# prstrive/SCGaussian

Hardware: AMD Instinct MI355X
Metric: train_iters_per_sec (higher is better)
Workload: dtype f32; 1 GPU; S2: 200000 Gaussians, 1008x756, SH degree 3, fwd+bwd per view (BASELINE configs[1] shape: LLFF-fern 3-view training, 200 k Gaussians @ 1008x756); gaussians=200000, width=1008, height=756, sh_degree=3, visible=174771, views=3, parallelism=single, ranks_seen=1, launched_by=single process, grad_bucket_bytes=0, grad_bucket_bytes_per_view=0

## Files before the change

### include/scg_raster.h

```cpp
#ifndef SCG_RASTER_H
#define SCG_RASTER_H

#include <stddef.h>
#include <stdint.h>

#ifndef SCG_API
#define SCG_API __attribute__((visibility("default")))
#endif

#ifdef __cplusplus
extern "C" {
#endif

#define SCG_TILE 16
#define SCG_SPLAT_FLOATS 12
#define SCG_DSPLAT_FLOATS 16
#define SCG_ABI_VERSION 10

enum {
    SCG_OK = 0,
    SCG_E_NULL = -1,
    SCG_E_RANGE = -2,
    SCG_E_EXCLUSIVE = -3,
    SCG_E_SCRATCH = -4,
// ... 1 lines not shown
};

typedef struct ScgFrame {
    int32_t P;
    int32_t sh_degree;
    int32_t sh_coeffs;
    int32_t width;
    int32_t height;
    float tanfovx;
    float tanfovy;
    float scale_modifier;
    int32_t prefiltered;
    int32_t debug;
    const float* viewmatrix;
    const float* projmatrix;
    const float* campos;
    const float* bg;
    const uint32_t* tile_cost_in;
    uint32_t* tile_cost_out;
    uint32_t* long_lists_out;
    const uint32_t* bwd_cost_in;
    uint32_t* bwd_cost_out;
    uint32_t* num_rendered_out;
} ScgFrame;


SCG_API const char* scg_last_error(void);
SCG_API int32_t scg_abi_version(void);
SCG_API size_t scg_struct_bytes(int32_t which );

SCG_API size_t scg_geometry_scratch_bytes(int32_t P);
SCG_API int scg_geometry_forward(const ScgFrame* frame,
                         const float* means3D, const float* opacities,
                         const float* shs, const float* colors_precomp,
                         const float* scales, const float* rotations, const float* cov3D_precomp,
                         float* splats, int32_t* radii, uint8_t* clamped,
                         uint32_t* rects, uint32_t* depth_keys, uint32_t* num_rendered_out,
                         void* scratch, size_t scratch_bytes, void* stream);

enum { SCG_BINNING_AUTO = 0, SCG_BINNING_GLOBAL_SORT = 1 };
SCG_API size_t scg_binning_scratch_bytes(int32_t P, int64_t num_rendered, int32_t width, int32_t height, int32_t algo);
SCG_API size_t scg_ranges_words(int32_t width, int32_t height);
SCG_API int32_t scg_binning_accepts_bound(int64_t num_rendered_bound, int32_t width, int32_t height, int32_t algo);
SCG_API int scg_binning(const ScgFrame* frame, int64_t num_rendered,
                const uint32_t* rects, const uint32_t* depth_keys,
                uint32_t* point_list, uint32_t* ranges, uint64_t* keys_sorted, int32_t algo,
// ... 160 lines not shown
```

### scgaussian_amd/_lib.py

```python
from __future__ import annotations

import ctypes as C
import os

import torch

_HERE = os.path.dirname(os.path.abspath(__file__))
LIB_PATH = os.environ.get("SCG_LIB_PATH") or os.path.join(_HERE, "libscg_raster.so")

ABI_VERSION = 10


class ScgFrame(C.Structure):
    _fields_ = [
        ("P", C.c_int32), ("sh_degree", C.c_int32), ("sh_coeffs", C.c_int32),
        ("width", C.c_int32), ("height", C.c_int32),
        ("tanfovx", C.c_float), ("tanfovy", C.c_float), ("scale_modifier", C.c_float),
        ("prefiltered", C.c_int32), ("debug", C.c_int32),
        ("viewmatrix", C.c_void_p), ("projmatrix", C.c_void_p), ("campos", C.c_void_p), ("bg", C.c_void_p),
        ("tile_cost_in", C.c_void_p), ("tile_cost_out", C.c_void_p), ("long_lists_out", C.c_void_p),
        ("bwd_cost_in", C.c_void_p), ("bwd_cost_out", C.c_void_p), ("num_rendered_out", C.c_void_p),
    ]


class ScgWorkspaceLayout(C.Structure):
    _fields_ = [(n, C.c_uint64) for n in ("splats", "rects", "depth_keys", "clamped", "point_list", "ranges", "final_T",
                                          "n_contrib", "bin_scratch", "total", "partial_words")]


class ScgStageEvents(C.Structure):
    _fields_ = [("begin", C.c_void_p * 3), ("end", C.c_void_p * 3)]


class ScgModelSet(C.Structure):
    _fields_ = [("count", C.c_int32)] + [(n, C.c_void_p) for n in ("zval", "rayo", "rayd", "xyz", "features_dc", "features_rest",
                                                                   "opacity", "scaling", "rotation")]


class ScgModel(C.Structure):
    _fields_ = [("ray", ScgModelSet), ("bg", ScgModelSet)]


class ScgModelGradSet(C.Structure):
    _fields_ = [(n, C.c_void_p) for n in ("zval", "xyz", "features_dc", "features_rest", "opacity", "scaling", "rotation")]
# ... 107 lines not shown
```

### scgaussian_amd/csrc/api.hip

```cpp
#include <stdarg.h>
#include <stdio.h>
#include <string.h>

#include "scg_common.h"
#include "scg_debug.h"

#include <atomic>
#include <chrono>
#include <thread>

namespace scg {

static thread_local char g_err[512] = "";

int fail(int code, const char* fmt, ...) {
    va_list ap;
    va_start(ap, fmt);
    vsnprintf(g_err, sizeof(g_err), fmt, ap);
    va_end(ap);
    return code;
}

int check_hip(hipError_t e, const char* what) {
    if (e == hipSuccess) return 0;
    snprintf(g_err, sizeof(g_err), "%s: %s (hipError %d)", what, hipGetErrorString(e), (int)e);
    return (int)e;
}

int validate_frame(const ScgFrame* f, bool need_bg) {
    if (!f) return fail(SCG_E_NULL, "frame is NULL");
    if (f->P < 0) return fail(SCG_E_RANGE, "P = %d < 0", f->P);
    if (f->width <= 0 || f->height <= 0 || f->width > 65535 * SCG_TILE || f->height > 65535 * SCG_TILE)
        return fail(SCG_E_RANGE, "image size %d x %d out of range", f->width, f->height);
    if (f->sh_degree < 0 || f->sh_degree > 3) return fail(SCG_E_RANGE, "sh_degree %d not in 0..3", f->sh_degree);
    if (!(f->tanfovx > 0.f) || !(f->tanfovy > 0.f)) return fail(SCG_E_RANGE, "tanfov must be positive");
    if (!f->viewmatrix || !f->projmatrix || !f->campos) return fail(SCG_E_NULL, "viewmatrix/projmatrix/campos is NULL");
    if (need_bg && !f->bg) return fail(SCG_E_NULL, "bg is NULL");
    return 0;
}

static inline size_t align_up(size_t v, size_t a) { return (v + a - 1) / a * a; }
static inline bool aligned16(const void* p) { return (reinterpret_cast<uintptr_t>(p) & 15u) == 0; }
static inline bool aligned64(const void* p) { return (reinterpret_cast<uintptr_t>(p) & 63u) == 0; }
int validate_model(const ScgFrame* f, const ScgModel* m);

static int validate_inputs(const ScgFrame* f, const float* means3D, const float* opacities, const float* shs,
                           const float* colors_precomp, const float* scales, const float* rotations,
                           const float* cov3D_precomp) {
    if (f->P == 0) return 0;
    if (!means3D || !opacities) return fail(SCG_E_NULL, "means3D/opacities is NULL");
    if ((shs == nullptr) == (colors_precomp == nullptr))
        return fail(SCG_E_EXCLUSIVE, "Please provide exactly one of either SHs or precomputed colors!");
    const bool has_sr = scales != nullptr && rotations != nullptr;
    if ((scales != nullptr) != (rotations != nullptr) || has_sr == (cov3D_precomp != nullptr))
        return fail(SCG_E_EXCLUSIVE,
                    "Please provide exactly one of either scale/rotation pair or precomputed 3D covariance!");
    if (shs && f->sh_coeffs < (f->sh_degree + 1) * (f->sh_degree + 1))
        return fail(SCG_E_RANGE, "sh_coeffs %d < (sh_degree+1)^2 = %d", f->sh_coeffs,
                    (f->sh_degree + 1) * (f->sh_degree + 1));
    if (rotations && !aligned16(rotations)) return fail(SCG_E_ALIGN, "rotations must be 16-byte aligned");
// ... 534 lines not shown
```

### scgaussian_amd/csrc/blend.hip

```cpp
#include "scg_common.h"
#include "tile_sort.h"

namespace scg {

constexpr float kHalfLog2e = 0.72134752044448170f;
typedef float f32x2 __attribute__((ext_vector_type(2)));
typedef float f32x4 __attribute__((ext_vector_type(4)));

__device__ __forceinline__ bool splat_hits_rect(const float4& a, const float4& b, float x0, float y0) {
    const float dx0 = x0 - a.x, dy0 = y0 - a.y, dx1 = dx0 + 7.0f, dy1 = dy0 + 7.0f;
    const float nx = __builtin_amdgcn_fmed3f(0.0f, dx0, dx1), ny = __builtin_amdgcn_fmed3f(0.0f, dy0, dy1);
    const float cb2 = a.w + a.w;
    const float ya = __builtin_amdgcn_fmed3f(b.w * nx, dy0, dy1);
    const float qa = nx * (a.z * nx + cb2 * ya) + b.x * ya * ya;
    const float xb = __builtin_amdgcn_fmed3f(-a.w * ny * __builtin_amdgcn_rcpf(a.z), dx0, dx1);
    const float qb = ny * (b.x * ny + cb2 * xb) + a.z * xb * xb;
    return !((qa > b.z) && (qb > b.z));
}

__device__ __forceinline__ int quadrant_workgroup(int wg, int n_tiles, const uint2* __restrict__ ranges, int& quad) {
    quad = (wg >> 3) & 3;
    const int per = (n_tiles + 7) >> 3;
    const uint32_t* order = reinterpret_cast<const uint32_t*>(ranges) + 2 * (size_t)n_tiles;
    return (int)order[(wg & 7) * per + (wg >> 5)];
// ... 11 lines not shown
                                             const float4* __restrict__ splats, float* __restrict__ out_color,
                                             float* __restrict__ out_depth, float* __restrict__ out_alpha,
                                             float* __restrict__ final_T, uint32_t* __restrict__ n_contrib) {
    const int tile_x = tile % f.gx, tile_y = tile / f.gx;
    const int qx0 = tile_x * kTile + (quad & 1) * 8, qy0 = tile_y * kTile + (quad >> 1) * 8;
    const int px = qx0 + (lane & 7), py = qy0 + (lane >> 3);
    const bool inside = (px < f.W) && (py < f.H);
    const float pxf = (float)px, pyf = (float)py;

    const int n = (int)(range.y - range.x);
    float T = inside ? 1.0f : -1.0f;
    int bgi0 = __builtin_amdgcn_readfirstlane(__builtin_bit_cast(int, f.bg[0]));
    int bgi1 = __builtin_amdgcn_readfirstlane(__builtin_bit_cast(int, f.bg[1]));
    int bgi2 = __builtin_amdgcn_readfirstlane(__builtin_bit_cast(int, f.bg[2]));
    asm volatile("" : "+s"(bgi0), "+s"(bgi1), "+s"(bgi2));
    f32x2 Crg = {0.f, 0.f}, Cbz = {0.f, 0.f};
    uint32_t last = 0;
    int n_blended = 0;
#ifndef SCG_FWD_TRIP_CXX
    const uint32_t lds_base = (uint32_t)reinterpret_cast<uintptr_t>(s_rec);
    const uint64_t exec_all = __builtin_amdgcn_read_exec();
#endif

    uint32_t id_next = 0;
    float4 ra, rb, rc;
    if (n > 0) {
        const uint32_t id0 = list[min(lane, n - 1)];
        id_next = list[min(kWave + lane, n - 1)];
        ra = splats[3 * (size_t)id0 + 0]; rb = splats[3 * (size_t)id0 + 1]; rc = splats[3 * (size_t)id0 + 2];
    }

    for (int base = 0; base < n; base += kWave) {
        if (__all(T < 0.0f)) break;
        const bool hit = (base + lane < n) && splat_hits_rect(ra, rb, (float)qx0, (float)qy0);
        if (hit) {
            *reinterpret_cast<float2*>(&s_rec[2 * kWave + lane]) = make_float2(ra.x, ra.y);
            s_rec[kWave + lane] = make_float4(kHalfLog2e * ra.z, 2.0f * kHalfLog2e * ra.w, kHalfLog2e * rb.x, rb.y);
            s_rec[lane] = rc;
        }
        uint64_t m = __ballot(hit);
        if (base + kWave < n) {
            ra = splats[3 * (size_t)id_next + 0]; rb = splats[3 * (size_t)id_next + 1];
            rc = splats[3 * (size_t)id_next + 2];
            id_next = list[min(base + 2 * kWave + lane, n - 1)];
        }
        wave_sync();

        n_blended += __builtin_popcountll(m);
#ifdef SCG_FWD_TRIP_CXX
        while (m) {
            const int j = __builtin_ctzll(m);
            asm("s_bitset0_b64 %0, %1" : "+s"(m) : "s"(j));
            const float2 c = *reinterpret_cast<const float2*>(&s_rec[2 * kWave + j]);
            const float4 q = s_rec[kWave + j];
            const float dx = c.x - pxf, dy = c.y - pyf;
            const float u = __builtin_fmaf(q.y, dy, q.x * dx);
            const float t = __builtin_fmaf(u, dx, (q.z * dy) * dy);
            const float alpha = fminf(kAlphaMax, q.w * __builtin_amdgcn_exp2f(-t));
            const float wgt = T * alpha;
            const float test_T = __builtin_fmaf(-T, alpha, T);
            if ((t >= 0.0f) && (alpha >= kAlphaMin)) {
                const bool contributes = test_T >= kTEps;
                const float T_prev = T;
// ... 245 lines not shown
        "v_cndmask_b32 %1, %3, %4, %20\n\t"
        "s_nop 1\n\t"
        "v_add_f32_dpp %0, %1, %5 quad_perm:[2,3,0,1] row_mask:0xf bank_mask:0xf"
        : "=&v"(y), "=&v"(t0), "=&v"(t1), "=&v"(t2), "=&v"(t3), "=&v"(t4), "=&v"(t5), "=&v"(t6), "=&v"(t7)
        : "v"(v0), "v"(v1), "v"(v2), "v"(v3), "v"(v4), "v"(v5), "v"(v6), "v"(v7), "v"(v8), "v"(v9), "s"(odd), "s"(hi));
    return y;
}

struct BwdLds {
    float4 a[kWave];
    float4 b[kWave];
    float4 c[kWave];
    __attribute__((aligned(16))) float w[kSlots * kWStride];
};

struct BwdPixel {
    float T, behind, dC0, dC1, dC2, dD, dA;
    uint32_t last;
};

__device__ __forceinline__ uint32_t top_chunk_index(int end) {
    return (uint32_t)min(((end - 1) / kWave) * kWave + (kWave - 1 - (int)threadIdx.x), end - 1);
}
__device__ __forceinline__ int backward_walk(BwdLds& L, const FrameDev& f, int tile, int quad, int first, int end,
                                              BwdPixel px, uint32_t list_begin, uint32_t id_top,
                                              const uint32_t* __restrict__ point_list,
                                              const float4* __restrict__ splats, float* __restrict__ dsplats) {
    const int lane = threadIdx.x;
    const int tile_x = tile % f.gx, tile_y = tile / f.gx;
    const int qx0 = tile_x * kTile + (quad & 1) * 8, qy0 = tile_y * kTile + (quad >> 1) * 8;
    const float pxf = (float)(qx0 + (lane & 7)), pyf = (float)(qy0 + (lane >> 3));
    float T = px.T, behind = px.behind;
    const float dC0 = px.dC0, dC1 = px.dC1, dC2 = px.dC2, dD = px.dD, dA = px.dA;
    const uint32_t last = px.last;

    const int row = lane >> 4, grp = lane & 15;
    float4 fc[4];
    {
        float4* tmp = reinterpret_cast<float4*>(L.w);
        __syncthreads();
        tmp[lane] = make_float4(dC0, dC1, dC2, dD);
        __syncthreads();
#pragma unroll
        for (int i = 0; i < 4; ++i) fc[i] = tmp[grp + 16 * i];
        __syncthreads();
    }
    const float gx_pix = (float)(qx0 + (grp & 7)), gy_pix = (float)(qy0 + (grp >> 3));
    float* w_store = L.w + 2 * lane;
// ... 47 lines not shown
            Gg = __builtin_fmaf(qw.y, fc[i].y, Gg);
            Bb = __builtin_fmaf(qw.y, fc[i].z, Bb);
            Dz = __builtin_fmaf(qw.y, fc[i].w, Dz);
        }
        const float Sx = dx * Sq, Sxx = dx * Sx, Sxy = dx * Sy;
        const float sum = row_reduce10(Sx, Sy, Dz, Sq,
                                       Sxx, Sxy, Syy, Rr,
                                       Gg, Bb, odd_lanes, hi_lanes);
        const uint32_t rec = my_id * (uint32_t)(SCG_DSPLAT_FLOATS * 4) + out_bytes;
        const uint64_t lanes = (rows >= kSlots) ? out_lanes : (out_lanes & ((1ull << (16 * rows)) - 1ull));
        asm volatile("s_mov_b64 exec, %[lanes]\n\t"
                     "global_atomic_add_f32 %[off], %[val], %[base]\n\t"
                     "s_mov_b64 exec, %[all]"
                     :: [lanes] "s"(lanes), [off] "v"(rec), [val] "v"(sum), [base] "s"(dsplats), [all] "s"(lanes_all)
                     : "memory");
        __builtin_amdgcn_fence(__ATOMIC_ACQ_REL, "wavefront");
        __builtin_amdgcn_wave_barrier();
    };

    float amax_s;
    asm volatile("s_mov_b32 %0, 0x3f7d70a4" : "=s"(amax_s));
    const int chunk_bot = first / kWave;
    uint32_t id = id_top;
    int n_trips = 0;
#ifdef SCG_FWD_TRIP_CXX
    float* w_ptr = w_store;
#else
    static_assert(offsetof(BwdLds, b) == 1024 && offsetof(BwdLds, c) == 2048 && kWStride * sizeof(float) == 512,
                  "the hand-written walk addresses the planes with immediate offsets");
    const uint32_t lds_rec = (uint32_t)reinterpret_cast<uintptr_t>(&L.a[0]);
    const uint32_t lds_w = (uint32_t)reinterpret_cast<uintptr_t>(w_store);
    const uint64_t row0 = 0x000000000000FFFFull, row1 = 0x00000000FFFF0000ull, row2 = 0x0000FFFF00000000ull,
                   row3 = 0xFFFF000000000000ull;
    typedef float f32x16 __attribute__((ext_vector_type(16)));
    const f32x16 fcv = {fc[0].x, fc[0].y, fc[0].z, fc[0].w, fc[1].x, fc[1].y, fc[1].z, fc[1].w,
                        fc[2].x, fc[2].y, fc[2].z, fc[2].w, fc[3].x, fc[3].y, fc[3].z, fc[3].w};
    const f32x4 dCv = {dC0, dC1, dC2, dD};
#endif
    for (int chunk = (end - 1) / kWave; chunk >= chunk_bot; --chunk) {
        const int base = chunk * kWave;
        const int k = base + (kWave - 1 - lane);
#ifdef SCG_FWD_TRIP_CXX
        const int first_j = base + (kWave - 1) - (int)last;
#else
        const int first_j = max(base + (kWave - 1) - (int)last, -1);
#endif
        const float4 a = splats[3 * (size_t)id + 0];
        const float4 b = splats[3 * (size_t)id + 1];
        const float4 c_rec = splats[3 * (size_t)id + 2];
        uint32_t id_next = id;
        if (chunk > chunk_bot) id_next = point_list[list_begin + (uint32_t)(k - kWave)];
        const bool hit = (k < end) && splat_hits_rect(a, b, (float)qx0, (float)qy0);
        if (hit) {
            L.a[lane] = make_float4(a.x, a.y, kHalfLog2e * a.z, 2.0f * kHalfLog2e * a.w);
            L.b[lane] = make_float4(kHalfLog2e * b.x, b.y, __builtin_bit_cast(float, id), 0.f);
            L.c[lane] = c_rec;
        }
        id = id_next;
        uint64_t m = __ballot(hit);
        n_trips += __builtin_popcountll(m);
        __builtin_amdgcn_s_waitcnt(0x0F70);
        __syncthreads();

#ifdef SCG_FWD_TRIP_CXX
        while (m) {
            const int j = __builtin_ctzll(m);
            asm("s_bitset0_b64 %0, %1" : "+s"(m) : "s"(j));
            const float4 a = L.a[j];
            const float4 b = L.b[j];
            const float4 c = L.c[j];
            asm("" ::"v"(b.w));
            const float dx = a.x - pxf, dy = a.y - pyf;
            float u = a.z * dx;
            asm("" : "+v"(u));
            u = __builtin_fmaf(a.w, dy, u);
            const float t = __builtin_fmaf(u, dx, (b.x * dy) * dy);
            const float oG = b.y * __builtin_amdgcn_exp2f(-t);
            const bool ok = (j > first_j) && (t >= 0.0f) && (oG >= kAlphaMin);
            if (__ballot(ok) == 0ull) continue;

            const float q0 = ok ? oG : 0.0f;
            const float alpha = __builtin_amdgcn_fmed3f(q0, 0.0f, amax_s);
// ... 215 lines not shown
    __shared__ BwdLds L;
    const int n_tiles = f.gx * f.gy;
    const int slots = tile_order_slots(n_tiles);
    const uint32_t* order_q = reinterpret_cast<const uint32_t*>(ranges) + 2 * (size_t)n_tiles + slots;
    const uint32_t entry = order_q[(size_t)(blockIdx.x & 7) * (4 * (slots >> 3)) + (blockIdx.x >> 3)];
    const int tile = (int)(entry >> 2), quad = (int)(entry & 3u);
    if (tile >= n_tiles) return;
    const int lane = threadIdx.x;
    const int px = (tile % f.gx) * kTile + (quad & 1) * 8 + (lane & 7), py = (tile / f.gx) * kTile + (quad >> 1) * 8 + (lane >> 3);
    const uint2 range = ranges[tile];
    const int n = (int)(range.y - range.x);
    const BwdPixel s = load_pixel_final(f, px, py, final_T, n_contrib, dL_dcolor, dL_ddepth, dL_dalpha);
    uint32_t mx = s.last;
#pragma unroll
    for (int off = 32; off > 0; off >>= 1) mx = max(mx, (uint32_t)__shfl_down((int)mx, off, kWave));
    const int limit = min(n, __builtin_amdgcn_readfirstlane((int)mx));
#ifdef SCG_PROBE_TIMELINE
    const uint32_t tp0 = (uint32_t)wall_clock64();
#endif
    if (limit <= 0) {
        if (f.bcost_out && lane == 0) f.bcost_out[4 * tile + quad] = 0u;
        return;
    }
    const int trips = backward_walk(L, f, tile, quad, 0, limit, s, range.x, point_list[range.x + top_chunk_index(limit)],
                                    point_list, splats, dsplats);
    if (f.bcost_out && lane == 0) f.bcost_out[4 * tile + quad] = (uint32_t)trips;
#ifdef SCG_PROBE_TIMELINE
    if (f.cost_out && lane == 0) {
        uint32_t* tl = f.cost_out + n_tiles + 65792 + 32768 + (size_t)(n_tiles + 8) * 40 + (size_t)blockIdx.x * 4;
        tl[0] = tp0; tl[1] = (uint32_t)wall_clock64(); tl[2] = ((uint32_t)min(trips, 65535) << 16) | (uint32_t)min(limit, 65535);
        tl[3] = 0xBAC00000u | (uint32_t)(4 * tile + quad);
    }
#endif
}

int launch_blend_backward(const FrameDev& f, const uint32_t* ranges, const uint32_t* point_list,
                          const float* splats, const float* final_T, const uint32_t* n_contrib,
                          const float* dL_dcolor, const float* dL_ddepth, const float* dL_dalpha,
                          float* dsplats, bool dsplats_prezeroed, hipStream_t stream, hipEvent_t started, hipEvent_t done) {
    if (!dsplats_prezeroed) {
        const int rc = check_hip(hipMemsetAsync(dsplats, 0, (size_t)f.P * SCG_DSPLAT_FLOATS * sizeof(float), stream),
                                 "dsplats memset");
        if (rc) return rc;
    }
    const int n_tiles = f.gx * f.gy;
    const int grid = ((n_tiles + 7) / 8) * 8 * 4;
    if (started || done) {
        hipExtLaunchKernelGGL(blend_backward_kernel, dim3(grid), dim3(kWave), 0u, stream, started, done, 0u, f,
// ... 12 lines not shown
```

### scgaussian_amd/csrc/scg_common.h

```cpp
#pragma once

#include <hip/hip_runtime.h>
#include <hip/hip_ext.h>
#include <stdint.h>

#include "../../include/scg_raster.h"

namespace scg {

constexpr int kWave = 64;
constexpr int kTile = SCG_TILE;
constexpr int kTilePix = kTile * kTile;
constexpr int kBlock = 256;

constexpr float kNearZ = 0.2f;
constexpr float kLowpass = 0.3f;
constexpr float kAlphaMin = 1.0f / 255.0f;
constexpr float kAlphaMax = 0.99f;
constexpr float kTEps = 1e-4f;

struct FrameDev {
    int P, D, M, W, H;
    int gx, gy;
    float tanfovx, tanfovy, focal_x, focal_y, limx, limy, mod;
    const float* view;
    const float* proj;
    const float* campos;
    const float* bg;
    const uint32_t* cost_in;
    uint32_t* cost_out;
    uint32_t* long_out;
    const uint32_t* bcost_in;
    uint32_t* bcost_out;
    uint32_t* nr_out;
};

inline FrameDev make_frame_dev(const ScgFrame* f) {
    FrameDev d;
    d.P = f->P; d.D = f->sh_degree; d.M = f->sh_coeffs; d.W = f->width; d.H = f->height;
    d.gx = (f->width + kTile - 1) / kTile;
    d.gy = (f->height + kTile - 1) / kTile;
    d.tanfovx = f->tanfovx; d.tanfovy = f->tanfovy;
    d.focal_x = (float)f->width / (2.0f * f->tanfovx);
    d.focal_y = (float)f->height / (2.0f * f->tanfovy);
    d.limx = 1.3f * f->tanfovx;
    d.limy = 1.3f * f->tanfovy;
    d.mod = f->scale_modifier;
    d.view = f->viewmatrix; d.proj = f->projmatrix; d.campos = f->campos; d.bg = f->bg;
    d.cost_in = f->tile_cost_in; d.cost_out = f->tile_cost_out; d.long_out = f->long_lists_out;
    d.bcost_in = f->bwd_cost_in; d.bcost_out = f->bwd_cost_out;
    d.nr_out = f->num_rendered_out;
    return d;
}

int fail(int code, const char* fmt, ...);
int check_hip(hipError_t e, const char* what);
int validate_frame(const ScgFrame* f, bool need_bg);

int launch_geometry_forward(const FrameDev& f, const float* means3D, const float* opacities, const float* shs,
                            const float* colors_precomp, const float* scales, const float* rotations,
                            const float* cov3D_precomp, float* splats, int32_t* radii, uint8_t* clamped,
                            uint32_t* rects, uint32_t* depth_keys, uint32_t* block_sums, hipStream_t stream);
int launch_geometry_backward(const FrameDev& f, const float* means3D, const float* opacities, const float* shs,
                             const float* colors_precomp, const float* scales, const float* rotations,
                             const float* cov3D_precomp, const int32_t* radii, const uint8_t* clamped,
                             const float* dsplats, float* dmeans3D, float* dmeans2D, float* dopac, float* dshs,
                             float* dcolors, float* dscales, float* drots, float* dcov3D, int flags ,
                             hipStream_t stream);
int launch_geometry_forward_model(const FrameDev& f, const ScgModel& m, float* splats, int32_t* radii, uint8_t* clamped,
                                  uint32_t* rects, uint32_t* depth_keys, uint32_t* block_sums, hipStream_t stream);
int launch_geometry_hist_model(const FrameDev& f, const ScgModel& m, float* splats, int32_t* radii, uint8_t* clamped,
                               uint32_t* rects, uint32_t* depth_keys, uint32_t* block_sums, int nblocks, uint32_t* table,
                               uint32_t* class_counts, uint32_t* len_hist, hipStream_t stream);
int launch_geometry_hist_binned_model(const FrameDev& f, int64_t R, const ScgModel& m, float* splats, int32_t* radii,
// ... 95 lines not shown
```

### scgaussian_amd/model_path.py

```python
from __future__ import annotations

import ctypes as C
import math
from typing import Optional

import torch

from . import _lib
from . import rasterizer as R
from ._lib import ScgModel, ScgModelGrads, check, ptr

_RAY = ("zval", "rayo", "rayd", "features_dc", "features_rest", "opacity", "scaling", "rotation")
_BG = ("bg_xyz", "bg_features_dc", "bg_features_rest", "bg_opacity", "bg_scaling", "bg_rotation")
ARG_NAMES = _RAY + _BG
_ARENA_ORDER = ("zval", "opacity", "scaling", "rotation", "features_dc", "bg_xyz", "bg_opacity", "bg_scaling", "bg_rotation",
                "bg_features_dc", "features_rest", "bg_features_rest")
_LAYOUTS = {}


class _ModelArgs:

    def __init__(self, tensors: dict):
        t = tensors
        self.tensors = tuple(t[n] for n in ARG_NAMES)
# ... 153 lines not shown
    fr = state["frame"]
    if fr.hints is not None and fr.hints.bcost is not None:
        fr.hints.bwritten = True
    H, W = fr.H, fr.W
    dL_dcolor = R._f32c(dL_dcolor, dev)
    if dL_dcolor is None:
        dL_dcolor = torch.zeros((3, H, W), dtype=torch.float32, device=dev)
    dL_ddepth = R._f32c(dL_ddepth, dev)
    dL_dalpha = R._f32c(dL_dalpha, dev)
    timer = timer or R._ACTIVE_TIMER
    with R._on_device(dev):
        stage_ev = timer.stage_events("backward") if isinstance(timer, R.StageTimer) else None
        stream = R._stream(dev)
        dsplats = state.get("dsplats_zeroed")
        state["dsplats_zeroed"] = None
        prezeroed = dsplats is not None
        keep = None
        if dsplats is None:
            keep = torch.empty((model.P, R.DSPLAT_FLOATS), dtype=torch.float32, device=dev)
            dsplats = keep.data_ptr()
        out = _grad_arena(model, into)
        d_means2D = d_means2D_out if d_means2D_out is not None else torch.empty((model.P, 3), dtype=torch.float32, device=dev)
        flags = 1 if into is not None else R._sh_tail_promise(out.get("_pooled"), (fr.c.sh_degree + 1) ** 2)
        check(lib.scg_backward_model(fr.ref, model.ref, radii.data_ptr(), state["cap"], state["ws"].data_ptr(),
                                     dL_dcolor.data_ptr(), ptr(dL_ddepth), ptr(dL_dalpha), dsplats, int(prezeroed),
                                     C.byref(out["_c"]), d_means2D.data_ptr(), flags, stage_ev, stream), "scg_backward_model")
    out = dict(out)
    out["means2D"] = d_means2D
    return out


class _RasterizeModel(torch.autograd.Function):
    @staticmethod
    def forward(ctx, means2D, *args):
        *tensors, raster_settings, model = args
        if model is None:
            model = _ModelArgs(dict(zip(ARG_NAMES, tensors)))
        needs_grad = any(ctx.needs_input_grad)
        fused = R.forward_fused(raster_settings, None, None, None, None, None, None, None, needs_grad, model=model)
        if fused is None:
            raise _lib.ScgError("the model path needs the tile-first binning (scg_binning_accepts_bound): check "
                                "model_path.supported(tensors, settings) first and render through the getters otherwise")
        color, radii, depth, alpha, state = fused
        state.pop("inputs")
        ctx.model = model
        ctx.fused_state = state
        ctx.raster_settings = raster_settings
        if needs_grad:
            ctx.save_for_backward(*model.tensors, radii)
# ... 106 lines not shown
```

### scgaussian_amd/rasterizer.py

```python
from __future__ import annotations

import contextlib
import math
import os
import ctypes as C
import threading
from typing import Callable, NamedTuple, Optional

import torch
import torch.nn as nn

from . import _lib
from ._lib import ScgFrame, check, ptr

SPLAT_FLOATS = 12
DSPLAT_FLOATS = 16
TILE = 16


class GaussianRasterizationSettings(NamedTuple):
    image_height: int
    image_width: int
    tanfovx: float
    tanfovy: float
# ... 114 lines not shown
        _LONG_POOL = (t, t.numpy(), t.data_ptr())
        _LONG_FREE.extend(range(_CAM_HINTS_MAX, -1, -1))
    _t, arr, base = _LONG_POOL
    if not _LONG_FREE:
        used = {h.slot for h in _CAM_HINTS.values()}
        _LONG_FREE.extend(i for i in range(_CAM_HINTS_MAX, -1, -1) if i not in used)
    i = _LONG_FREE.pop()
    view = arr[2 * i: 2 * i + 2]
    view[:] = -1
    return i, view, base + 8 * i


def _release_long_words(h):
    if h.slot is not None:
        _LONG_FREE.append(h.slot)
        h.slot = h.long_np = h.long_ptr = None


TILE_COST_HINT = True
BWD_ORDER_HINT = True
SKIP_IDLE_RARE_SORT = True
SPLIT_LONG_LISTS = True
RARE_8WAVE = True


def _rare_options(words) -> int:
    if words is None or words[0] < 0:
        return 0
    if words[0] == 0:
        return 8 if SKIP_IDLE_RARE_SORT else 0
    if RARE_8WAVE and SPLIT_LONG_LISTS and words[1] > 0:
        return 16 | 32
    return 0


def _frame_for(settings: GaussianRasterizationSettings, P: int, M: int, device, forward: bool = False) -> _Frame:
    small = (settings.viewmatrix, settings.projmatrix, settings.campos, settings.bg)
    for t in small:
        if not (isinstance(t, torch.Tensor) and t.dtype == torch.float32 and t.device == device and t.is_contiguous()
                and t.numel() > 0):
            return _Frame(settings, P, M, device)
    key = (small[0].data_ptr(), small[1].data_ptr(), small[2].data_ptr(), small[3].data_ptr(),
           settings.image_height, settings.image_width, settings.tanfovx, settings.tanfovy,
           settings.scale_modifier, settings.sh_degree, settings.prefiltered, settings.debug, P, M, device.index)
    fr = _FRAME_CACHE.get(key)
    if fr is None:
# ... 304 lines not shown
        pinned = spec.take(gscratch) if speculative else None
        with timer("geometry_forward"):
            check(lib.scg_geometry_forward(fr.ref, ptr(means3D), ptr(opacities), ptr(shs), ptr(colors_precomp),
                                           ptr(scales), ptr(rotations), ptr(cov3D_precomp), ga.ptr(0), ptr(radii),
                                           ga.ptr(3), ga.ptr(1), ga.ptr(2), None if speculative else ga.ptr(5),
                                           pinned.ptr if speculative else ga.ptr(4), gscratch, stream),
                  "scg_geometry_forward")
        if speculative:
            pinned.torch_event().record()
            R = None
            cap = int(guess)
        else:
            nr = ga.view(5, (1,), torch.int32)
            R = int(nr.item()) & 0xFFFFFFFF
            cap = R

        img = torch.empty((5, H, W), dtype=torch.float32, device=dev)
        color, depth, alpha = img[0:3], img[3:4], img[4:5]

        dsplats = torch.empty((P, DSPLAT_FLOATS), dtype=torch.float32, device=dev) if prepare_backward and P > 0 else None

        def bin_and_blend(capacity):
            scratch_bytes = lib.scg_binning_scratch_bytes(P, capacity, W, H, binning_algo)
            ba = _Arena([capacity * 4, lib.scg_ranges_words(W, H) * 4, H * W * 4, H * W * 4, scratch_bytes,
                         capacity * 8 if want_keys else 0], dev)
            with timer("binning"):
                check(lib.scg_binning(fr.ref, capacity, ga.ptr(1), ga.ptr(2), ba.ptr(0), ba.ptr(1),
                                      ba.ptr(5) if want_keys else None, binning_algo, ba.ptr(4), scratch_bytes, stream),
                      "scg_binning")
            with timer("blend_forward"):
                check(lib.scg_blend_forward(fr.ref, ba.ptr(1), ba.ptr(0), ga.ptr(0), ptr(color), ptr(depth), ptr(alpha),
                                            ba.ptr(2), ba.ptr(3), ptr(dsplats), stream), "scg_blend_forward")
            return ba

        ba = bin_and_blend(cap)
        out = _LazyViews(dict(color=color, depth=depth, alpha=alpha, radii=radii, num_rendered=R, dsplats_zeroed=dsplats,
                              arenas=(ga, ba), capacity=cap, n_tiles=fr.n_tiles, hw=(H, W), P=P, frame=fr,
                              ptrs=dict(splats=ga.ptr(0), clamped=ga.ptr(3), point_list=ba.ptr(0), ranges=ba.ptr(1),
                                        final_T=ba.ptr(2), n_contrib=ba.ptr(3)),
                              inputs=(means3D, opacities, shs, colors_precomp, scales, rotations, cov3D_precomp)),
                         want_keys)
        if speculative:
            pinned.torch_event().synchronize()
            R = int(pinned.np[: (P + 255) // 256].sum(dtype="int64"))
            spec.give_back(pinned)
            if R > cap:
                ba = bin_and_blend(R)
                cap = R
                out["arenas"] = (ga, ba)
                out["capacity"] = cap
                out["ptrs"].update(point_list=ba.ptr(0), ranges=ba.ptr(1), final_T=ba.ptr(2), n_contrib=ba.ptr(3))
            out["num_rendered"] = R
        if capacity_hint is None:
            spec.hint[key] = _next_capacity(spec.hint.get(key), R)
    return out


class _LazyViews(dict):

    _SPECS = {
        "splats": (0, 0, lambda d: (d["P"], SPLAT_FLOATS), torch.float32),
        "rects": (0, 1, lambda d: (d["P"], 2), torch.int32),
        "depth_keys": (0, 2, lambda d: (d["P"],), torch.int32),
        "clamped": (0, 3, lambda d: (d["P"],), torch.uint8),
        "point_list": (1, 0, lambda d: (d["num_rendered"],), torch.int32),
        "ranges": (1, 1, lambda d: (d["n_tiles"], 2), torch.int32),
        "final_T": (1, 2, lambda d: d["hw"], torch.float32),
        "n_contrib": (1, 3, lambda d: d["hw"], torch.int32),
        "keys_sorted": (1, 5, lambda d: (d["num_rendered"],), torch.int64),
    }

    def __init__(self, d, want_keys):
        super().__init__(d)
        self._want_keys = want_keys
# ... 101 lines not shown
    means3D, opacities, shs, colors_precomp, scales, rotations, cov3D_precomp = inputs
    dev = means3D.device
    P = means3D.shape[0]
    M = shs.shape[1] if shs is not None else 0
    fr = saved.get("frame") if isinstance(saved, dict) else None
    if fr is None:
        fr = _frame_for(settings, P, M, dev)
    if fr.hints is not None and fr.hints.bcost is not None:
        fr.hints.bwritten = True
    H, W = fr.H, fr.W
    dL_dcolor = _f32c(dL_dcolor, dev)
    if dL_dcolor is None:
        dL_dcolor = torch.zeros((3, H, W), dtype=torch.float32, device=dev)
    dL_ddepth = _f32c(dL_ddepth, dev)
    dL_dalpha = _f32c(dL_dalpha, dev)
    with _on_device(dev):
        stream = _stream(dev)
        dsplats = saved.pop("dsplats_zeroed", None) if isinstance(saved, dict) else None
        prezeroed = dsplats is not None
        if dsplats is None:
            dsplats = torch.empty((P, DSPLAT_FLOATS), dtype=torch.float32, device=dev)
        with timer("blend_backward"):
            sp = saved["ptrs"]
            check(lib.scg_blend_backward(fr.ref, sp["ranges"], sp["point_list"], sp["splats"], sp["final_T"],
                                         sp["n_contrib"], ptr(dL_dcolor), ptr(dL_ddepth), ptr(dL_dalpha),
                                         ptr(dsplats), int(prezeroed), stream), "scg_blend_backward")
        out = _grad_outputs(inputs, into, d_means2D_out, dev)
        flags = 1 if into is not None else _sh_tail_promise(out.get("_pooled"), (fr.c.sh_degree + 1) ** 2)
        with timer("geometry_backward"):
            check(lib.scg_geometry_backward(fr.ref, ptr(means3D), ptr(opacities), ptr(shs), ptr(colors_precomp),
                                            ptr(scales), ptr(rotations), ptr(cov3D_precomp), ptr(saved["radii"]),
                                            saved["ptrs"]["clamped"], ptr(dsplats), ptr(out["means3D"]),
                                            ptr(out["means2D"]), ptr(out["opacities"]), ptr(out["shs"]),
                                            ptr(out["colors_precomp"]), ptr(out["scales"]), ptr(out["rotations"]),
                                            ptr(out["cov3D_precomp"]), flags, stream),
                  "scg_geometry_backward")
    if want_dsplats:
        out["dsplats"] = dsplats
    return out


NO_HOST_READ = False
_CAPTURE_RECORD = None


@contextlib.contextmanager
def no_host_read(enabled: bool = True):
    global NO_HOST_READ
    prev, NO_HOST_READ = NO_HOST_READ, bool(enabled)
# ... 56 lines not shown
        fr = _frame_for(settings, P, M, dev, forward=True)
        _SPEC_STATS["one_call_forwards"] += 1
        if fr.c.tile_cost_in:
            _SPEC_STATS["tile_cost_hints"] += 1
        if fr.c.bwd_cost_in:
            _SPEC_STATS["bwd_order_hints"] += 1
        timer = timer or _ACTIVE_TIMER
        with _on_device(dev):
            stage_ev = timer.stage_events("forward") if isinstance(timer, StageTimer) else None
            stream = _stream(dev)
            ev = None if EVENTLESS_WAIT else pinned.event_handle()
            img = torch.empty((5, H, W), dtype=torch.float32, device=dev)
            radii = torch.empty((P,), dtype=torch.int32, device=dev)
            ds_bytes = (P * DSPLAT_FLOATS * 4 + 64) if prepare_backward else 0
            ip = img.data_ptr()
            hw4 = H * W * 4
            if model is None:
                inputs = (means3D, opacities, shs, colors_precomp, scales, rotations, cov3D_precomp)
                in_ptrs = tuple(None if t is None else t.data_ptr() for t in inputs)
            else:
                inputs = model.tensors
            cw = None
            while True:
                ws = torch.empty((plan.total + ds_bytes + (plan.partial_bytes + 256 if no_read else 0),), dtype=torch.uint8,
                                 device=dev)
                wp = ws.data_ptr()
                dsplats = ((wp + plan.total + 63) & ~63) if prepare_backward else None
                options = (0 if FUSED_SORT else 1) | (0 if FUSED_HIST else 2) | (0 if prepare_backward else 4) | \
                    _rare_options(fr.long_np) | (64 if (ev is None and not no_read) else 0)
                if fr.long_np is not None and fr.long_np[0] >= 0 and not plan.sorts_in_blend(lib, options):
                    fr.long_np[:] = -1
                    options &= ~(8 | 16 | 32)
                if no_read:
                    cw = _count_word(cap, P, ckey, dev.index)
                    fr.c.num_rendered_out = cw.ptr
                    sums, ev = (wp + plan.total + ds_bytes + 255) & ~255, None
                else:
                    fr.c.num_rendered_out = None
                    sums = pinned.ptr
                try:
                    if model is None:
                        check(lib.scg_forward(fr.ref, *in_ptrs, cap, wp, plan.total, radii.data_ptr(), ip,
                                              ip + 3 * hw4, ip + 4 * hw4, sums, ev,
                                              dsplats, options, stage_ev,
                                              stream), "scg_forward")
                    else:
                        check(lib.scg_forward_model(fr.ref, model.ref, cap, wp, plan.total, radii.data_ptr(), ip,
                                                    ip + 3 * hw4, ip + 4 * hw4, sums, ev, dsplats, options, stage_ev,
                                                    stream), "scg_forward_model")
                finally:
                    fr.c.num_rendered_out = None
                if no_read:
                    _OVERFLOW["renders"] += 1
                    if capturing:
                        cw.captured = True
                        (_CAPTURE_RECORD if _CAPTURE_RECORD is not None else _ANON_CAPTURED).append(cw)
                    else:
                        spec.pending.setdefault(ckey, []).append(cw)
                    R = None
                    break
                R = lib.scg_wait_num_rendered(ev, pinned.ptr, P)
                if R < 0:
                    check(int(R), "scg_wait_num_rendered")
                if R <= cap:
                    break
                _SPEC_STATS["overflow_retries"] += 1
                cap = _capacity_for(R)
                plan = spec.plan(lib, P, W, H, cap)
                if not plan.accepts:
                    spec.cam_hint.pop((W, H, cam), None)
                    spec.hint.pop((P, W, H), None)
                    spec.give_back(pinned)
                    return None
                stage_ev = None
            if R is not None:
                nxt = _next_capacity(cap, R)
                spec.hint[(P, W, H)] = nxt
                spec.cam_hint.pop((W, H, cam), None)
                spec.cam_hint[(W, H, cam)] = (nxt, R, P)
            for table in (spec.hint, spec.cam_hint):
                if len(table) > 1024:
                    for k in list(table)[:128]:
                        del table[k]
        state = {"ws": ws, "cap": cap, "plan": plan, "frame": fr, "dsplats_zeroed": dsplats, "num_rendered": R,
                 "inputs": inputs, "has_backward_state": bool(prepare_backward), "count_word": cw}
        if pinned is not None:
            spec.give_back(pinned)
        return img[0:3], radii, img[3:4], img[4:5], state
    except BaseException:
        try:
            if not capturing:
                torch.cuda.current_stream(dev).synchronize()
        except Exception:
            pass
        if pinned is not None:
            _QUARANTINE.append(pinned)
        raise


def backward_fused(inputs, radii, state, dL_dcolor, dL_ddepth, dL_dalpha, timer: Optional[Callable] = None, into=None,
                   d_means2D_out=None):
    lib = _lib.load()
    if not state.get("has_backward_state", True):
        raise _lib.ScgError("this forward ran without backward state (prepare_backward=False -> scg_forward's "
                            "SCG_FORWARD_NO_BACKWARD_STATE: final_T / n_contrib were not written): it cannot be differentiated")
    means3D = inputs[0]
    dev = means3D.device
    fr = state["frame"]
    if fr.hints is not None and fr.hints.bcost is not None:
        fr.hints.bwritten = True
    H, W = fr.H, fr.W
    dL_dcolor = _f32c(dL_dcolor, dev)
    if dL_dcolor is None:
        dL_dcolor = torch.zeros((3, H, W), dtype=torch.float32, device=dev)
    dL_ddepth = _f32c(dL_ddepth, dev)
    dL_dalpha = _f32c(dL_dalpha, dev)
    timer = timer or _ACTIVE_TIMER
    with _on_device(dev):
        stage_ev = timer.stage_events("backward") if isinstance(timer, StageTimer) else None
        stream = _stream(dev)
        dsplats = state.get("dsplats_zeroed")
        state["dsplats_zeroed"] = None
        prezeroed = dsplats is not None
        keep = None
        if dsplats is None:
            keep = torch.empty((means3D.shape[0], DSPLAT_FLOATS), dtype=torch.float32, device=dev)
            dsplats = keep.data_ptr()
        out = _grad_outputs(inputs, into, d_means2D_out, dev)
        flags = 1 if into is not None else _sh_tail_promise(out.get("_pooled"), (fr.c.sh_degree + 1) ** 2)
        check(lib.scg_backward(fr.ref, *(None if t is None else t.data_ptr() for t in inputs), radii.data_ptr(),
                               state["cap"], state["ws"].data_ptr(), dL_dcolor.data_ptr(), ptr(dL_ddepth), ptr(dL_dalpha),
                               dsplats, int(prezeroed), out["means3D"].data_ptr(), out["means2D"].data_ptr(),
                               out["opacities"].data_ptr(), ptr(out["shs"]), ptr(out["colors_precomp"]), ptr(out["scales"]),
                               ptr(out["rotations"]), ptr(out["cov3D_precomp"]), flags, stage_ev, stream),
              "scg_backward")
    return out


def grad_arena(params):
    if not params or params[0].grad is None:
        return None
    st = params[0].grad.untyped_storage()
    base = st.data_ptr()
    begin, end, covered = None, 0, 0
    for p in params:
        g = p.grad
        if g is None or g.dtype != torch.float32 or not g.is_contiguous() or g.untyped_storage().data_ptr() != base:
            return None
        off = g.storage_offset()
        begin = off if begin is None else min(begin, off)
        end = max(end, off + g.numel())
        covered += g.numel()
    if end * 4 > st.nbytes() or (end - begin) - covered > 3 * len(params):
        return None
    return torch.empty((0,), dtype=torch.float32, device=params[0].grad.device).set_(st, begin, (end - begin,))


class _RasterizeGaussians(torch.autograd.Function):
# ... 206 lines not shown
```

Before: 4327 iters/s.

## Cache per-quad hit ballots in forward blend and reuse them in backward walk

The forward blend now writes each 64-splat chunk's per-quad hit ballot into a new hit_masks buffer. The backward walk reads these masks instead of reloading every splat and re-testing it against the quad rectangle. It loads splat records only for lanes that hit and skips chunks with no hits at all. This adds a workspace allocation, an extra global store per chunk in forward and an ABI struct field, and it depends on the forward and backward chunk indexing matching exactly.

```diff
diff --git a/include/scg_raster.h b/include/scg_raster.h
--- a/include/scg_raster.h
+++ b/include/scg_raster.h
@@ -47,6 +47,7 @@
     const uint32_t* bwd_cost_in;
     uint32_t* bwd_cost_out;
     uint32_t* num_rendered_out;
+    uint64_t* hit_masks;
 } ScgFrame;
 
 
diff --git a/scgaussian_amd/_lib.py b/scgaussian_amd/_lib.py
--- a/scgaussian_amd/_lib.py
+++ b/scgaussian_amd/_lib.py
@@ -20,6 +20,7 @@
         ("viewmatrix", C.c_void_p), ("projmatrix", C.c_void_p), ("campos", C.c_void_p), ("bg", C.c_void_p),
         ("tile_cost_in", C.c_void_p), ("tile_cost_out", C.c_void_p), ("long_lists_out", C.c_void_p),
         ("bwd_cost_in", C.c_void_p), ("bwd_cost_out", C.c_void_p), ("num_rendered_out", C.c_void_p),
+        ("hit_masks", C.c_void_p),
     ]
 
 
diff --git a/scgaussian_amd/csrc/api.hip b/scgaussian_amd/csrc/api.hip
--- a/scgaussian_amd/csrc/api.hip
+++ b/scgaussian_amd/csrc/api.hip
@@ -36,6 +36,7 @@
     if (!(f->tanfovx > 0.f) || !(f->tanfovy > 0.f)) return fail(SCG_E_RANGE, "tanfov must be positive");
     if (!f->viewmatrix || !f->projmatrix || !f->campos) return fail(SCG_E_NULL, "viewmatrix/projmatrix/campos is NULL");
     if (need_bg && !f->bg) return fail(SCG_E_NULL, "bg is NULL");
+    if (reinterpret_cast<uintptr_t>(f->hit_masks) & 7u) return fail(SCG_E_ALIGN, "hit_masks must be 8-byte aligned");
     return 0;
 }
 
diff --git a/scgaussian_amd/csrc/blend.hip b/scgaussian_amd/csrc/blend.hip
--- a/scgaussian_amd/csrc/blend.hip
+++ b/scgaussian_amd/csrc/blend.hip
@@ -57,6 +57,7 @@
     const uint64_t exec_all = __builtin_amdgcn_read_exec();
 #endif
 
+    uint64_t* hm = (final_T && f.hit_masks) ? f.hit_masks + 4 * (size_t)hit_mask_slot(range.x, tile) + quad : nullptr;
     uint32_t id_next = 0;
     float4 ra, rb, rc;
     if (n > 0) {
@@ -74,6 +75,7 @@
             s_rec[lane] = rc;
         }
         uint64_t m = __ballot(hit);
+        if (hm && lane == 0) hm[4 * (base >> 6)] = m;
         if (base + kWave < n) {
             ra = splats[3 * (size_t)id_next + 0]; rb = splats[3 * (size_t)id_next + 1];
             rc = splats[3 * (size_t)id_next + 2];
@@ -365,8 +367,13 @@
 __device__ __forceinline__ uint32_t top_chunk_index(int end) {
     return (uint32_t)min(((end - 1) / kWave) * kWave + (kWave - 1 - (int)threadIdx.x), end - 1);
 }
+__device__ __forceinline__ uint64_t uniform64(uint64_t v) {
+    return ((uint64_t)(uint32_t)__builtin_amdgcn_readfirstlane((int)(v >> 32)) << 32) |
+           (uint64_t)(uint32_t)__builtin_amdgcn_readfirstlane((int)(uint32_t)v);
+}
 __device__ __forceinline__ int backward_walk(BwdLds& L, const FrameDev& f, int tile, int quad, int first, int end,
                                               BwdPixel px, uint32_t list_begin, uint32_t id_top,
+                                              const uint64_t* __restrict__ hm, uint64_t m_top,
                                               const uint32_t* __restrict__ point_list,
                                               const float4* __restrict__ splats, float* __restrict__ dsplats) {
     const int lane = threadIdx.x;
@@ -460,6 +467,7 @@
     asm volatile("s_mov_b32 %0, 0x3f7d70a4" : "=s"(amax_s));
     const int chunk_bot = first / kWave;
     uint32_t id = id_top;
+    uint64_t m_cur = m_top;
     int n_trips = 0;
 #ifdef SCG_FWD_TRIP_CXX
     float* w_ptr = w_store;
@@ -483,19 +491,44 @@
 #else
         const int first_j = max(base + (kWave - 1) - (int)last, -1);
 #endif
-        const float4 a = splats[3 * (size_t)id + 0];
-        const float4 b = splats[3 * (size_t)id + 1];
-        const float4 c_rec = splats[3 * (size_t)id + 2];
-        uint32_t id_next = id;
-        if (chunk > chunk_bot) id_next = point_list[list_begin + (uint32_t)(k - kWave)];
-        const bool hit = (k < end) && splat_hits_rect(a, b, (float)qx0, (float)qy0);
-        if (hit) {
-            L.a[lane] = make_float4(a.x, a.y, kHalfLog2e * a.z, 2.0f * kHalfLog2e * a.w);
-            L.b[lane] = make_float4(kHalfLog2e * b.x, b.y, __builtin_bit_cast(float, id), 0.f);
-            L.c[lane] = c_rec;
-        }
-        id = id_next;
-        uint64_t m = __ballot(hit);
+        uint64_t m;
+        if (hm) {
+            m = __builtin_bitreverse64(uniform64(m_cur));
+            if (base + kWave > end) m &= ~0ull << (base + kWave - end);
+            uint32_t id_next = id;
+            if (chunk > chunk_bot) {
+                id_next = point_list[list_begin + (uint32_t)(k - kWave)];
+                m_cur = hm[4 * (chunk - 1)];
+            }
+            if (m == 0ull) {
+                id = id_next;
+                __builtin_amdgcn_s_waitcnt(0x0F70);
+                continue;
+            }
+            if ((m >> lane) & 1ull) {
+                const float4 a = splats[3 * (size_t)id + 0];
+                const float4 b = splats[3 * (size_t)id + 1];
+                const float4 c_rec = splats[3 * (size_t)id + 2];
+                L.a[lane] = make_float4(a.x, a.y, kHalfLog2e * a.z, 2.0f * kHalfLog2e * a.w);
+                L.b[lane] = make_float4(kHalfLog2e * b.x, b.y, __builtin_bit_cast(float, id), 0.f);
+                L.c[lane] = c_rec;
+            }
+            id = id_next;
+        } else {
+            const float4 a = splats[3 * (size_t)id + 0];
+            const float4 b = splats[3 * (size_t)id + 1];
+            const float4 c_rec = splats[3 * (size_t)id + 2];
+            uint32_t id_next = id;
+            if (chunk > chunk_bot) id_next = point_list[list_begin + (uint32_t)(k - kWave)];
+            const bool hit = (k < end) && splat_hits_rect(a, b, (float)qx0, (float)qy0);
+            if (hit) {
+                L.a[lane] = make_float4(a.x, a.y, kHalfLog2e * a.z, 2.0f * kHalfLog2e * a.w);
+                L.b[lane] = make_float4(kHalfLog2e * b.x, b.y, __builtin_bit_cast(float, id), 0.f);
+                L.c[lane] = c_rec;
+            }
+            id = id_next;
+            m = __ballot(hit);
+        }
         n_trips += __builtin_popcountll(m);
         __builtin_amdgcn_s_waitcnt(0x0F70);
         __syncthreads();
@@ -757,8 +790,12 @@
         if (f.bcost_out && lane == 0) f.bcost_out[4 * tile + quad] = 0u;
         return;
     }
+    const uint64_t* hm = f.hit_masks ? f.hit_masks + 4 * (size_t)__builtin_amdgcn_readfirstlane((int)hit_mask_slot(range.x, tile)) +
+                                           __builtin_amdgcn_readfirstlane(quad)
+                                     : nullptr;
+    const uint64_t m_top = hm ? hm[4 * ((limit - 1) / kWave)] : 0ull;
     const int trips = backward_walk(L, f, tile, quad, 0, limit, s, range.x, point_list[range.x + top_chunk_index(limit)],
-                                    point_list, splats, dsplats);
+                                    hm, m_top, point_list, splats, dsplats);
     if (f.bcost_out && lane == 0) f.bcost_out[4 * tile + quad] = (uint32_t)trips;
 #ifdef SCG_PROBE_TIMELINE
     if (f.cost_out && lane == 0) {
diff --git a/scgaussian_amd/csrc/scg_common.h b/scgaussian_amd/csrc/scg_common.h
--- a/scgaussian_amd/csrc/scg_common.h
+++ b/scgaussian_amd/csrc/scg_common.h
@@ -33,7 +33,10 @@
     const uint32_t* bcost_in;
     uint32_t* bcost_out;
     uint32_t* nr_out;
+    uint64_t* hit_masks;
 };
+
+__host__ __device__ inline uint32_t hit_mask_slot(uint32_t range_begin, int tile) { return (range_begin >> 6) + (uint32_t)tile; }
 
 inline FrameDev make_frame_dev(const ScgFrame* f) {
     FrameDev d;
@@ -50,6 +53,7 @@
     d.cost_in = f->tile_cost_in; d.cost_out = f->tile_cost_out; d.long_out = f->long_lists_out;
     d.bcost_in = f->bwd_cost_in; d.bcost_out = f->bwd_cost_out;
     d.nr_out = f->num_rendered_out;
+    d.hit_masks = f->hit_masks;
     return d;
 }
 
diff --git a/scgaussian_amd/model_path.py b/scgaussian_amd/model_path.py
--- a/scgaussian_amd/model_path.py
+++ b/scgaussian_amd/model_path.py
@@ -199,9 +199,13 @@
         out = _grad_arena(model, into)
         d_means2D = d_means2D_out if d_means2D_out is not None else torch.empty((model.P, 3), dtype=torch.float32, device=dev)
         flags = 1 if into is not None else R._sh_tail_promise(out.get("_pooled"), (fr.c.sh_degree + 1) ** 2)
-        check(lib.scg_backward_model(fr.ref, model.ref, radii.data_ptr(), state["cap"], state["ws"].data_ptr(),
-                                     dL_dcolor.data_ptr(), ptr(dL_ddepth), ptr(dL_dalpha), dsplats, int(prezeroed),
-                                     C.byref(out["_c"]), d_means2D.data_ptr(), flags, stage_ev, stream), "scg_backward_model")
+        fr.c.hit_masks = state.get("hit_masks")
+        try:
+            check(lib.scg_backward_model(fr.ref, model.ref, radii.data_ptr(), state["cap"], state["ws"].data_ptr(),
+                                         dL_dcolor.data_ptr(), ptr(dL_ddepth), ptr(dL_dalpha), dsplats, int(prezeroed),
+                                         C.byref(out["_c"]), d_means2D.data_ptr(), flags, stage_ev, stream), "scg_backward_model")
+        finally:
+            fr.c.hit_masks = None
     out = dict(out)
     out["means2D"] = d_means2D
     return out
diff --git a/scgaussian_amd/rasterizer.py b/scgaussian_amd/rasterizer.py
--- a/scgaussian_amd/rasterizer.py
+++ b/scgaussian_amd/rasterizer.py
@@ -160,6 +160,11 @@
 SKIP_IDLE_RARE_SORT = True
 SPLIT_LONG_LISTS = True
 RARE_8WAVE = True
+HIT_MASKS = True
+
+
+def _hit_mask_bytes(capacity: int, n_tiles: int) -> int:
+    return ((int(capacity) >> 6) + n_tiles + 1) * 32
 
 
 def _rare_options(words) -> int:
@@ -510,22 +515,28 @@
 
         def bin_and_blend(capacity):
             scratch_bytes = lib.scg_binning_scratch_bytes(P, capacity, W, H, binning_algo)
+            masks = prepare_backward and HIT_MASKS
             ba = _Arena([capacity * 4, lib.scg_ranges_words(W, H) * 4, H * W * 4, H * W * 4, scratch_bytes,
-                         capacity * 8 if want_keys else 0], dev)
+                         capacity * 8 if want_keys else 0, _hit_mask_bytes(capacity, fr.n_tiles) if masks else 0], dev)
+            ba.hit_masks = ba.ptr(6) if masks else None
             with timer("binning"):
                 check(lib.scg_binning(fr.ref, capacity, ga.ptr(1), ga.ptr(2), ba.ptr(0), ba.ptr(1),
                                       ba.ptr(5) if want_keys else None, binning_algo, ba.ptr(4), scratch_bytes, stream),
                       "scg_binning")
             with timer("blend_forward"):
-                check(lib.scg_blend_forward(fr.ref, ba.ptr(1), ba.ptr(0), ga.ptr(0), ptr(color), ptr(depth), ptr(alpha),
-                                            ba.ptr(2), ba.ptr(3), ptr(dsplats), stream), "scg_blend_forward")
+                fr.c.hit_masks = ba.hit_masks
+                try:
+                    check(lib.scg_blend_forward(fr.ref, ba.ptr(1), ba.ptr(0), ga.ptr(0), ptr(color), ptr(depth), ptr(alpha),
+                                                ba.ptr(2), ba.ptr(3), ptr(dsplats), stream), "scg_blend_forward")
+                finally:
+                    fr.c.hit_masks = None
             return ba
 
         ba = bin_and_blend(cap)
         out = _LazyViews(dict(color=color, depth=depth, alpha=alpha, radii=radii, num_rendered=R, dsplats_zeroed=dsplats,
                               arenas=(ga, ba), capacity=cap, n_tiles=fr.n_tiles, hw=(H, W), P=P, frame=fr,
                               ptrs=dict(splats=ga.ptr(0), clamped=ga.ptr(3), point_list=ba.ptr(0), ranges=ba.ptr(1),
-                                        final_T=ba.ptr(2), n_contrib=ba.ptr(3)),
+                                        final_T=ba.ptr(2), n_contrib=ba.ptr(3), hit_masks=ba.hit_masks),
                               inputs=(means3D, opacities, shs, colors_precomp, scales, rotations, cov3D_precomp)),
                          want_keys)
         if speculative:
@@ -537,7 +548,8 @@
                 cap = R
                 out["arenas"] = (ga, ba)
                 out["capacity"] = cap
-                out["ptrs"].update(point_list=ba.ptr(0), ranges=ba.ptr(1), final_T=ba.ptr(2), n_contrib=ba.ptr(3))
+                out["ptrs"].update(point_list=ba.ptr(0), ranges=ba.ptr(1), final_T=ba.ptr(2), n_contrib=ba.ptr(3),
+                                   hit_masks=ba.hit_masks)
             out["num_rendered"] = R
         if capacity_hint is None:
             spec.hint[key] = _next_capacity(spec.hint.get(key), R)
@@ -685,9 +697,13 @@
             dsplats = torch.empty((P, DSPLAT_FLOATS), dtype=torch.float32, device=dev)
         with timer("blend_backward"):
             sp = saved["ptrs"]
-            check(lib.scg_blend_backward(fr.ref, sp["ranges"], sp["point_list"], sp["splats"], sp["final_T"],
-                                         sp["n_contrib"], ptr(dL_dcolor), ptr(dL_ddepth), ptr(dL_dalpha),
-                                         ptr(dsplats), int(prezeroed), stream), "scg_blend_backward")
+            fr.c.hit_masks = sp.get("hit_masks")
+            try:
+                check(lib.scg_blend_backward(fr.ref, sp["ranges"], sp["point_list"], sp["splats"], sp["final_T"],
+                                             sp["n_contrib"], ptr(dL_dcolor), ptr(dL_ddepth), ptr(dL_dalpha),
+                                             ptr(dsplats), int(prezeroed), stream), "scg_blend_backward")
+            finally:
+                fr.c.hit_masks = None
         out = _grad_outputs(inputs, into, d_means2D_out, dev)
         flags = 1 if into is not None else _sh_tail_promise(out.get("_pooled"), (fr.c.sh_degree + 1) ** 2)
         with timer("geometry_backward"):
@@ -790,9 +806,11 @@
                 inputs = model.tensors
             cw = None
             while True:
-                ws = torch.empty((plan.total + ds_bytes + (plan.partial_bytes + 256 if no_read else 0),), dtype=torch.uint8,
-                                 device=dev)
+                sums_bytes = plan.partial_bytes + 256 if no_read else 0
+                hm_bytes = (_hit_mask_bytes(cap, fr.n_tiles) + 256) if (prepare_backward and HIT_MASKS) else 0
+                ws = torch.empty((plan.total + ds_bytes + sums_bytes + hm_bytes,), dtype=torch.uint8, device=dev)
                 wp = ws.data_ptr()
+                hit_masks = ((wp + plan.total + ds_bytes + sums_bytes + 255) & ~255) if hm_bytes else None
                 dsplats = ((wp + plan.total + 63) & ~63) if prepare_backward else None
                 options = (0 if FUSED_SORT else 1) | (0 if FUSED_HIST else 2) | (0 if prepare_backward else 4) | \
                     _rare_options(fr.long_np) | (64 if (ev is None and not no_read) else 0)
@@ -806,6 +824,7 @@
                 else:
                     fr.c.num_rendered_out = None
                     sums = pinned.ptr
+                fr.c.hit_masks = hit_masks
                 try:
                     if model is None:
                         check(lib.scg_forward(fr.ref, *in_ptrs, cap, wp, plan.total, radii.data_ptr(), ip,
@@ -818,6 +837,7 @@
                                                     stream), "scg_forward_model")
                 finally:
                     fr.c.num_rendered_out = None
+                    fr.c.hit_masks = None
                 if no_read:
                     _OVERFLOW["renders"] += 1
                     if capturing:
@@ -851,7 +871,7 @@
                     for k in list(table)[:128]:
                         del table[k]
         state = {"ws": ws, "cap": cap, "plan": plan, "frame": fr, "dsplats_zeroed": dsplats, "num_rendered": R,
-                 "inputs": inputs, "has_backward_state": bool(prepare_backward), "count_word": cw}
+                 "inputs": inputs, "has_backward_state": bool(prepare_backward), "count_word": cw, "hit_masks": hit_masks}
         if pinned is not None:
             spec.give_back(pinned)
         return img[0:3], radii, img[3:4], img[4:5], state
@@ -896,12 +916,16 @@
             dsplats = keep.data_ptr()
         out = _grad_outputs(inputs, into, d_means2D_out, dev)
         flags = 1 if into is not None else _sh_tail_promise(out.get("_pooled"), (fr.c.sh_degree + 1) ** 2)
-        check(lib.scg_backward(fr.ref, *(None if t is None else t.data_ptr() for t in inputs), radii.data_ptr(),
-                               state["cap"], state["ws"].data_ptr(), dL_dcolor.data_ptr(), ptr(dL_ddepth), ptr(dL_dalpha),
-                               dsplats, int(prezeroed), out["means3D"].data_ptr(), out["means2D"].data_ptr(),
-                               out["opacities"].data_ptr(), ptr(out["shs"]), ptr(out["colors_precomp"]), ptr(out["scales"]),
-                               ptr(out["rotations"]), ptr(out["cov3D_precomp"]), flags, stage_ev, stream),
-              "scg_backward")
+        fr.c.hit_masks = state.get("hit_masks")
+        try:
+            check(lib.scg_backward(fr.ref, *(None if t is None else t.data_ptr() for t in inputs), radii.data_ptr(),
+                                   state["cap"], state["ws"].data_ptr(), dL_dcolor.data_ptr(), ptr(dL_ddepth), ptr(dL_dalpha),
+                                   dsplats, int(prezeroed), out["means3D"].data_ptr(), out["means2D"].data_ptr(),
+                                   out["opacities"].data_ptr(), ptr(out["shs"]), ptr(out["colors_precomp"]), ptr(out["scales"]),
+                                   ptr(out["rotations"]), ptr(out["cov3D_precomp"]), flags, stage_ev, stream),
+                  "scg_backward")
+        finally:
+            fr.c.hit_masks = None
     return out
 
 
```

Result: no change. 4352 iters/s, median of 6 (+0.6%).
